# Gorilla-Lab-SCUT/frustum-convnet

Hardware: AMD Instinct MI355X
Metric: frustums/sec (train fwd+bwd) KITTI-car B=32 N=1024 (higher is better)
Workload: dtype f32 (fp32 operands split into two 16-bit parts, 3 MFMAs per product, fp32 accumulate); 1 GPU; cfgs/det_sample.yaml KITTI-car, batch=32/GPU, Npoint=1024, L=(280,140,70,35), train fwd+bwd+Adam; global_batch=32, parallelism=dp1

## Files before the change

frustum_convnet_amd/_native.py:

```python
import ctypes
import os

_HERE = os.path.dirname(os.path.abspath(__file__))
LIB_PATH = os.path.join(_HERE, os.environ.get("FCN_LIB_NAME", "libfcn_hip.so"))

c_fp = ctypes.c_void_p

BN_RUNNING = 0
BN_TRAIN = 1
BN_FROZEN = 2


class PnDesc(ctypes.Structure):
    _fields_ = [("B", ctypes.c_int32), ("N", ctypes.c_int32), ("L", ctypes.c_int32), ("K", ctypes.c_int32),
                ("C1", ctypes.c_int32), ("C2", ctypes.c_int32), ("C3", ctypes.c_int32),
                ("nvec", ctypes.c_int32), ("training", ctypes.c_int32),
                ("eps", ctypes.c_float), ("momentum", ctypes.c_float), ("nlc", ctypes.c_int32),
                ("precision", ctypes.c_int32), ("grouped", ctypes.c_int32)]


CN_MAXLEV = 5
CN_MAXLAYER = 18


# ... 4 lines not shown
                ("precision", ctypes.c_int32), ("nlev", ctypes.c_int32), ("c1", ctypes.c_int32)]


class CnParams(ctypes.Structure):
    _fields_ = [("W", c_fp * CN_MAXLAYER), ("gamma", c_fp * CN_MAXLAYER), ("beta", c_fp * CN_MAXLAYER),
                ("running_mean", c_fp * CN_MAXLAYER), ("running_var", c_fp * CN_MAXLAYER),
                ("num_batches_tracked", c_fp * CN_MAXLAYER), ("bias", c_fp)]


class CnWs(ctypes.Structure):
    _fields_ = [("y", c_fp), ("dz", c_fp), ("wp", c_fp), ("bn", c_fp), ("stat", c_fp), ("bstat", c_fp),
                ("coef", c_fp), ("partial", c_fp), ("oh64", c_fp), ("flags", c_fp)]


class PnParams(ctypes.Structure):
    _fields_ = [("W", c_fp * 3), ("gamma", c_fp * 3), ("beta", c_fp * 3),
                ("running_mean", c_fp * 3), ("running_var", c_fp * 3), ("num_batches_tracked", c_fp * 3)]


class PnWs(ctypes.Structure):
    _fields_ = [("woff", c_fp), ("ent", c_fp), ("ewin", c_fp), ("tiles", c_fp), ("y2", c_fp), ("y3", c_fp), ("amax", c_fp),
                ("stat", c_fp), ("bn", c_fp), ("gmax", c_fp), ("dy3", c_fp), ("dz2", c_fp), ("bstat", c_fp),
                ("coef", c_fp), ("partial", c_fp), ("nsplit", ctypes.c_int32), ("gmom", c_fp), ("wenc", c_fp), ("flags", c_fp), ("pkey", c_fp),
                ("partial_both", ctypes.c_int32)]


class PnInferWs(ctypes.Structure):
    _fields_ = [("w1f", c_fp), ("wenc", c_fp), ("shift", c_fp)]


class InpDesc(ctypes.Structure):
    _fields_ = [("B", ctypes.c_int32), ("N", ctypes.c_int32), ("pt_stride", ctypes.c_int32), ("L", ctypes.c_int32 * 4),
                ("stride", ctypes.c_double * 4), ("max_depth", ctypes.c_double),
                ("random_flip", ctypes.c_int32), ("random_shift", ctypes.c_int32)]


class Inp5Desc(ctypes.Structure):
    _fields_ = [("B", ctypes.c_int32), ("N", ctypes.c_int32), ("pt_stride", ctypes.c_int32), ("L", ctypes.c_int32 * 5),
                ("stride", ctypes.c_double * 5), ("max_depth", ctypes.c_double),
                ("random_flip", ctypes.c_int32), ("random_shift", ctypes.c_int32)]


class InpRefineDesc(ctypes.Structure):
    _fields_ = [("B", ctypes.c_int32), ("N", ctypes.c_int32), ("pt_stride", ctypes.c_int32), ("Lpad", ctypes.c_int32 * 4),
                ("stride", ctypes.c_double * 4), ("random_flip", ctypes.c_int32), ("random_shift", ctypes.c_int32)]


# ... 225 lines not shown
```

frustum_convnet_amd/csrc/group_compact.hip:

```cpp
#include "fcn_common.h"
#include "pn_pack.h"

#define GC_T 256
#define GC_WAVES (GC_T / 64)
#ifndef GC_WPB
#define GC_WPB 16
#endif
#define GC_MAX_SCALES 8
#define GC_LDS_MAX_PTS 8192
#define GC_MOM 12

struct GcScale {
    const float *ref;
    float dis_z;
    int L, K, C1, C2, C3;
    int32_t *woff, *ewin, *tiles, *cnt;
    float4 *ent;
    unsigned short *ghits;
    double *stat;
    double *gmom;
    const float *W1, *gamma, *beta;
    float *rmean, *rvar;
    int64_t *nbt;
    float *bn1;
// ... 4 lines not shown
    PackArgs pk[GC_MAX_SCALES];
    const float *pc;
    int B, N, use_lds;
    int batch_stats;
    float eps, momentum;
    int fold;
};

#define GE_T 1024
#define GE_WAVES (GE_T / 64)

__device__ __forceinline__ GcScale gc_pick(const GcArgs &a, int z)
{
    GcScale S = a.s[0];
#pragma unroll
    for (int q = 1; q < GC_MAX_SCALES; ++q)
        if (z == q) S = a.s[q];
    return S;
}


__device__ __forceinline__ void gc_fold_bn1(const GcArgs &a, const GcScale &S, const double *mo, int tid, int nthr)
{
    const double M = (double)a.B * (double)S.L * (double)S.K;
    for (int c = tid; c < S.C1; c += nthr) {
        double mean, var;
        if (a.batch_stats) {
            const double iM = 1.0 / M;
            const double mx = mo[1] * iM, my = mo[2] * iM, mz = mo[3] * iM;
            const double cxx = mo[4] * iM - mx * mx, cxy = mo[5] * iM - mx * my, cxz = mo[6] * iM - mx * mz;
            const double cyy = mo[7] * iM - my * my, cyz = mo[8] * iM - my * mz, czz = mo[9] * iM - mz * mz;
            const double w0 = S.W1[3 * c], w1 = S.W1[3 * c + 1], w2 = S.W1[3 * c + 2];
            mean = w0 * mx + w1 * my + w2 * mz;
            var = w0 * (cxx * w0 + cxy * w1 + cxz * w2) + w1 * (cxy * w0 + cyy * w1 + cyz * w2) +
                  w2 * (cxz * w0 + cyz * w1 + czz * w2);
            if (var < 0.0) var = 0.0;
            if (S.rmean) {
                S.rmean[c] = (float)((1.0 - a.momentum) * S.rmean[c] + a.momentum * mean);
                S.rvar[c] = (float)((1.0 - a.momentum) * S.rvar[c] + a.momentum * var * (M / (M - 1.0)));
                if (c == 0 && S.nbt) S.nbt[0] += 1;
            }
        } else {
            mean = S.rmean[c];
            var = S.rvar[c];
        }
        const double rstd = fcn_rsqrt64(var + (double)a.eps);
        const double sc = (double)S.gamma[c] * rstd;
        S.bn1[c] = (float)sc;
        S.bn1[S.C1 + c] = (float)((double)S.beta[c] - mean * sc);
        S.bn1[2 * S.C1 + c] = (float)mean;
        S.bn1[3 * S.C1 + c] = (float)rstd;
    }
}

__global__ __launch_bounds__(GC_T) void gc_hits_kernel(GcArgs a)
{
    FCN_DYN_LDS(unsigned char, smem);
    const int tid = threadIdx.x, lane = tid & 63, wave = tid >> 6;
    const int b = blockIdx.y;
    const GcScale S = gc_pick(a, (int)blockIdx.z);
    const int L = S.L, K = S.K, N = a.N;
    {
        PackArgs P = a.pk[0];
#pragma unroll
        for (int q = 1; q < GC_MAX_SCALES; ++q)
            if ((int)blockIdx.z == q) P = a.pk[q];
        if (P.wenc) pn_pack_range(P, ((int)blockIdx.y * (int)gridDim.x + (int)blockIdx.x) * GC_T + tid, (int)(gridDim.x * gridDim.y) * GC_T);
    }
    if ((int)blockIdx.x * GC_WPB >= L) return;
    float *zs = (float *)smem;
    const float *pz = a.pc + (int64_t)b * 3 * N + 2 * (int64_t)N;
    if (a.use_lds) {
        for (int i = tid; i < N; i += GC_T) zs[i] = pz[i];
        __syncthreads();
// ... 256 lines not shown
```

frustum_convnet_amd/csrc/pn_pack.h:

```cpp
#pragma once
#include "gemm_tile.h"

__host__ __device__ inline int64_t pn_wenc_off(int img, int C1, int C2, int C3)
{
    const int64_t a = (int64_t)C2 * C1, b = (int64_t)C3 * C2;
    return img == 0 ? 0 : (img == 1 ? a : (img == 2 ? a + b : 2 * a + b));
}
__host__ __device__ inline int64_t pn_wenc_floats(int C1, int C2, int C3) { return 2 * ((int64_t)C2 * C1 + (int64_t)C3 * C2); }

template <int MM>
__device__ __forceinline__ void pn_pack_item(const float *__restrict__ W, int COUT, int CIN, bool grad, int t, u32x4 *__restrict__ img)
{
    const int NC = grad ? CIN : COUT;
    const int n = t % NC, r = t / NC, kb = r & 3, c = r >> 2;
    float x[8];
    if (!grad) {
        const v4f a = ldg4(W + (int64_t)n * CIN + c * KC + 8 * kb), b = ldg4(W + (int64_t)n * CIN + c * KC + 8 * kb + 4);
        x[0] = a.x; x[1] = a.y; x[2] = a.z; x[3] = a.w; x[4] = b.x; x[5] = b.y; x[6] = b.z; x[7] = b.w;
    } else {
#pragma unroll
        for (int j = 0; j < 8; ++j) x[j] = W[(int64_t)(c * KC + 8 * kb + j) * CIN + n];
    }
    u32x4 hi, lo;
    enc8<MM>(x, hi, lo);
    img[((int64_t)c * 8 + kb) * NC + n] = hi;
    img[((int64_t)c * 8 + 4 + kb) * NC + n] = lo;
}

struct PackArgs {
    const float *W2, *W3;
    float *wenc;
    int C1, C2, C3, precision;
};

__device__ __forceinline__ void pn_pack_range(const PackArgs &a, int first, int step)
{
    const int n2 = a.C2 * a.C1 / 8, n3 = a.C3 * a.C2 / 8;
    u32x4 *F2 = (u32x4 *)(a.wenc + pn_wenc_off(0, a.C1, a.C2, a.C3)), *F3 = (u32x4 *)(a.wenc + pn_wenc_off(1, a.C1, a.C2, a.C3));
    u32x4 *G2 = (u32x4 *)(a.wenc + pn_wenc_off(2, a.C1, a.C2, a.C3)), *G3 = (u32x4 *)(a.wenc + pn_wenc_off(3, a.C1, a.C2, a.C3));
    const int mmf = FCN_MM_OF(a.precision, true), mmb = FCN_MM_OF(a.precision, false);
    for (int t = first; t < 2 * (n2 + n3); t += step) {
        const bool grad = t >= n2 + n3;
        const int u = grad ? t - (n2 + n3) : t;
        const bool l3 = u >= n2;
        const int v = l3 ? u - n2 : u;
        const float *W = l3 ? a.W3 : a.W2;
        const int COUT = l3 ? a.C3 : a.C2, CIN = l3 ? a.C2 : a.C1;
        u32x4 *img = grad ? (l3 ? G3 : G2) : (l3 ? F3 : F2);
        const int mm = grad ? mmb : mmf;
        if (mm == MM_F32) pn_pack_item<MM_F32>(W, COUT, CIN, grad, v, img);
        else if (mm == MM_F16X3) pn_pack_item<MM_F16X3>(W, COUT, CIN, grad, v, img);
// ... 6 lines not shown
```

frustum_convnet_amd/csrc/pointnet_fwd.hip:

```cpp
#define FCN_TUNING_PNF
#include "gemm_tile.h"

#define LDT 129
#define MAXC 512
#ifndef FCN_WIDE_TILES
#define FCN_WIDE_TILES 0
#endif
#ifndef FCN_C3_BIG
#define FCN_C3_BIG 1
#endif
#ifndef FCN_FWD_EPI_DIRECT
#define FCN_FWD_EPI_DIRECT 0
#endif

__global__ void bn1_finalize_kernel(const double *__restrict__ mom, const float *__restrict__ W1,
                                    const float *__restrict__ gamma, const float *__restrict__ beta,
                                    float *rmean, float *rvar, int64_t *nbt, int C, int batch_stats,
                                    float eps, float momentum, double M, float *__restrict__ bn)
{
    const int c = blockIdx.x * blockDim.x + threadIdx.x;
    if (c >= C) return;
    double mean, var;
    if (batch_stats) {
        const double mx = mom[1] / M, my = mom[2] / M, mz = mom[3] / M;
// ... 110 lines not shown
    const float4 *ent;
    const int32_t *woff;
    const int32_t *tiles;
    const float *aprev;
    const float *bn_in;
    const float *W1;
    const u32x4 *Wenc;
    int32_t *flags;
    float *y;
    double *stat;
    int save_y;
    int L, cap, CIN, COUT, tps;
    const double *stat_in;
    int rep_stride;
    const float *gamma_in, *beta_in;
    float *rmean_in, *rvar_in;
    int64_t *nbt_in;
    float *bn_pub;
    double M;
    float eps, momentum;
    const int32_t *ewin;
    unsigned long long *pkey;
    const float *gamma_out;
};

__device__ __forceinline__ void fwd_bn_in(const FwdArgs &a, int i, bool pub, float &fs, float &ft, bool have = false, double s1 = 0.0,
                                          double s2 = 0.0)
{
    const int C = a.CIN;
    double mean, var;
    if (a.stat_in) {
        const double invM = 1.0 / a.M;
        if (!have) {
            s1 = fcn_rep_sum(a.stat_in + i, a.rep_stride);
            s2 = fcn_rep_sum(a.stat_in + C + i, a.rep_stride);
        }
        mean = s1 * invM;
        var = s2 * invM - mean * mean;
        if (var < 0.0) var = 0.0;
    } else {
        mean = a.rmean_in[i];
        var = a.rvar_in[i];
    }
    const double rstd = fcn_rsqrt64(var + (double)a.eps);
    const double sc = (double)a.gamma_in[i] * rstd;
    fs = (float)sc;
    ft = (float)((double)a.beta_in[i] - mean * sc);
    if (pub) {
        a.bn_pub[i] = fs; a.bn_pub[C + i] = ft; a.bn_pub[2 * C + i] = (float)mean; a.bn_pub[3 * C + i] = (float)rstd;
        if (a.stat_in && a.rmean_in) {
            a.rmean_in[i] = (float)((1.0 - a.momentum) * a.rmean_in[i] + a.momentum * mean);
            a.rvar_in[i] = (float)((1.0 - a.momentum) * a.rvar_in[i] + a.momentum * var * (a.M / (a.M - 1.0)));
            if (i == 0 && a.nbt_in) a.nbt_in[0] += 1;
        }
    }
}

template <int MM, int MODE, int NT, int WN, int MT = 2, int POOL = 0>
__global__ __launch_bounds__(128 * WN) __attribute__((amdgpu_waves_per_eu(MT == 1 ? 4 : 3, 4))) void fwd_gemm_kernel(FwdArgs a)
{
    constexpr int NTHR = 128 * WN;
    constexpr int TM = 64 * MT;
    constexpr int SUB = 128 / TM;
    constexpr int TN = 32 * NT * WN;
    constexpr int LDRA = KbTile<TM>::LDR, LDRB = KbTile<TN>::LDR;
    constexpr int NA4 = TM * 8 / NTHR;
    constexpr int NB = TN * 8 / NTHR;
    constexpr int KBT = 4 * TM / NTHR;
    constexpr int OPU4 = KbTile<TM>::U4 + KbTile<TN>::U4, EPU4 = (NTHR / 64) * EP_FLOATS / 4;
    constexpr int LDSU4 = OPU4 > EPU4 ? OPU4 : EPU4;
    __shared__ u32x4 lds4[LDSU4];
    __shared__ __attribute__((aligned(16))) float tS[MAXC];
    __shared__ __attribute__((aligned(16))) float sS[MODE == 0 ? 3 * MAXC : MAXC];
    __shared__ float wS[TM];
    __shared__ int winS[POOL ? TM : 1], insS[POOL ? 64 : 1];
    u32x4 *Ab = lds4, *Bb = lds4 + KbTile<TM>::U4;

    const int tid = threadIdx.x, lane = tid & 63, wave = tid >> 6;
    const int l31 = lane & 31, lh = lane >> 5;
    const int wm = wave / WN, wn = wave % WN;
    const int ny = a.COUT / TN;
    if constexpr (MODE == 1) {
        if (blockIdx.x == 0 && a.gamma_in) {
            for (int i = tid; i < a.CIN; i += NTHR) {
                float fs, ft;
                fwd_bn_in(a, i, true, fs, ft);
            }
        }
    }
    double q1[FCN_STAT_REP], q2[FCN_STAT_REP];
    const bool early = FCN_EARLY_STATS && MODE == 1 && a.gamma_in && a.stat_in && tid < a.CIN;
    if constexpr (MODE == 1) {
        if (early) {
#pragma unroll
            for (int r = 0; r < FCN_STAT_REP; ++r) {
                q1[r] = a.stat_in[(int64_t)r * a.rep_stride + tid];
                q2[r] = a.stat_in[(int64_t)r * a.rep_stride + a.CIN + tid];
            }
        }
        FCN_LOAD_FENCE();
    }
    const int xt = fcn_xcd_tile(blockIdx.x, SUB * a.tiles[0] * ny);
    if (xt < 0) return;
    const int bxi = xt / ny, byi = xt % ny;
    const int lt = bxi / SUB, sub = bxi % SUB;
    const int code = a.tiles[4 + lt];
    const int b = code / a.tps, t = code % a.tps;
    const int nent = a.woff[(int64_t)b * (a.L + 1) + a.L];
    const int row0 = t * 128 + sub * TM;
    const int nvalid = min(TM, nent - row0);
    if (nvalid <= 0) return;
    const int64_t grow0 = (int64_t)b * a.cap + row0;
    const int n0 = byi * TN;
    const int CIN = a.CIN, COUT = a.COUT;

    PNF_DECL;
    u32x4 rw[NB];
    v4f ra[MODE == 1 ? NA4 : 1];
    const u32x4 *wsrc = a.Wenc + n0 + (tid % TN) + (int64_t)(tid / TN) * COUT;
    auto load_chunk = [&](int c) __attribute__((always_inline)) {
        if constexpr (MODE == 1) {
            if (!((FCN_X & 1) && c > 0))
#pragma unroll
            for (int i = 0; i < NA4; ++i) {
                const int f = tid + NTHR * i;
                const int r = f >> 3, kq = f & 7;
                ra[i] = lds4e<MM>(a.aprev, ((int)grow0 + min(r, nvalid - 1)) * CIN + c * KC + 4 * kq);
            }
        }
        if (!((FCN_X & 2) && c > 0))
#pragma unroll
        for (int i = 0; i < NB; ++i) rw[i] = ldgu4(wsrc + ((int64_t)c * 8 + i * (NTHR / TN)) * COUT);
    };
    load_chunk(0);

    for (int i = tid; i < CIN; i += NTHR) {
        float s, t;
        if (MODE == 1 && a.gamma_in) {
            if (early && i == tid) {
                double s1 = q1[0], s2 = q2[0];
#pragma unroll
                for (int r = 1; r < FCN_STAT_REP; ++r) { s1 += q1[r]; s2 += q2[r]; }
                fwd_bn_in(a, i, false, s, t, true, s1, s2);
            } else {
                fwd_bn_in(a, i, false, s, t);
            }
        } else {
            s = a.bn_in[i];
            t = a.bn_in[CIN + i];
        }
        tS[i] = t;
        if constexpr (MODE == 0) {
            sS[3 * i] = s * a.W1[3 * i];
            sS[3 * i + 1] = s * a.W1[3 * i + 1];
            sS[3 * i + 2] = s * a.W1[3 * i + 2];
        } else {
            sS[i] = s;
        }
    }
    if (tid < TM) wS[tid] = (tid < nvalid) ? a.ent[grow0 + tid].w : 0.f;
    int pw = -1, plo = 0, phi = 0;
// ... 31 lines not shown
                const v4f s4 = *(const v4f *)(sS + c * KC + 4 * kq), t4 = *(const v4f *)(tS + c * KC + 4 * kq);
                const float z0 = fcn_relu_keep(fmaf(s4.x, ra[i].x, t4.x), kp), z1 = fcn_relu_keep(fmaf(s4.y, ra[i].y, t4.y), kp);
                const float z2 = fcn_relu_keep(fmaf(s4.z, ra[i].z, t4.z), kp), z3 = fcn_relu_keep(fmaf(s4.w, ra[i].w, t4.w), kp);
                kb_store4<MM_ENC_A, LDRA>(Aq, r, kq, z0, z1, z2, z3);
            }
        } else {
            const int part = tid / TM;
#pragma unroll
            for (int q = 0; q < KBT; ++q) {
                const int kb = part * KBT + q;
                float z[8];
#pragma unroll
                for (int j = 0; j < 8; ++j) {
                    const int kk = c * KC + 8 * kb + j;
                    const float zz = l1_pre(&sS[3 * kk], tS[kk], ux, uy, uz);
                    z[j] = fcn_relu_keep(zz, r0keep);
                }
                u32x4 hi, lo;
                enc8<MM_ENC_A>(z, hi, lo);
                Aq[kb * LDRA + r0] = hi;
                Aq[(4 + kb) * LDRA + r0] = lo;
            }
        }
#pragma unroll
        for (int i = 0; i < NB; ++i) {
            const int f = tid + NTHR * i;
            Bq[(f / TN) * LDRB + (f % TN)] = rw[i];
        }
    };

    PNF_ADD(0);
    for (int c = 0; c < nchunk; ++c) {
        if (!((FCN_X & 4) && c > 0)) stage_chunk(c, Ab, Bb);
        PNF_ADD(2);
        __syncthreads();
        PNF_ADD(3);
        if (c + 1 < nchunk) load_chunk(c + 1);
        PNF_ADD(1);
        if (!(FCN_X & 8)) mma_chunk_kb<MM, MT, NT, LDRA, LDRB>(Ab, Bb, wm * 32 * MT, wn * 32 * NT, acc);
        PNF_ADD(4);
        __syncthreads();
        PNF_ADD(3);
    }

    if (FCN_X & 16) { if (acc[0][0][0] == 123.456f) a.y[0] = 0.f; return; }
    bool bad = false;
    const bool store_y = !POOL || a.save_y;
#if FCN_FWD_EPI_DIRECT
#pragma unroll
    for (int mt = 0; mt < MT; ++mt)
// ... 373 lines not shown
        int ao[2];
#pragma unroll
        for (int e = 0; e < 2; ++e) {
            int row;
            const float y = fcn_pool_key_value(hi[e], lo[e], g[e], row);
            const float u = fmaf(s[e], y, t[e]);
            const bool pos = live && (hi[e] | lo[e]) != 0u && u > 0.f;
            fo[e] = pos ? u : 0.f;
            ao[e] = pos ? row : -1;
            yo[e] = y;
            if (ywin && y3 && g[e] == 0.f && pos) {
                const int64_t yi = ((int64_t)b * cap + row) * C3 + c + e;
                yo[e] = s16 ? __uint_as_float((unsigned)((const unsigned short *)y3)[yi] << 16) : ((const float *)y3)[yi];
            }
        }
        *(v2f *)(feat + o) = v2f{fo[0], fo[1]};
        if (amax) { amax[o] = ao[0]; amax[o + 1] = ao[1]; }
        if (ywin) *(v2f *)(ywin + o) = v2f{yo[0], yo[1]};
    }
}

static inline unsigned pad8(unsigned n) { return (n + 7u) / 8u * 8u; }

template <int MM, int MODE, int POOL>
static int launch_fwd_gemm_mm(const FwdArgs &a, int B, hipStream_t st)
{
    const unsigned nt = (unsigned)(B * a.tps);
    if (FCN_WIDE_TILES && a.COUT % 256 == 0) {
        hipLaunchKernelGGL((fwd_gemm_kernel<MM, MODE, 2, 4, 2, POOL>), dim3(pad8(nt * (a.COUT / 256))), dim3(512), 0, st, a);
    } else if (!FCN_C3_BIG && MODE == 1 && a.COUT >= 512 && a.COUT % 128 == 0) {
        hipLaunchKernelGGL((fwd_gemm_kernel<MM, MODE, 2, 2, 1, POOL>), dim3(pad8(2 * nt * (a.COUT / 128))), dim3(256), 0, st, a);
    } else if (a.COUT % 128 == 0) {
        hipLaunchKernelGGL((fwd_gemm_kernel<MM, MODE, 2, 2, 2, POOL>), dim3(pad8(nt * (a.COUT / 128))), dim3(256), 0, st, a);
    } else {
        hipLaunchKernelGGL((fwd_gemm_kernel<MM, MODE, 1, 2, 2, POOL>), dim3(pad8(nt * (a.COUT / 64))), dim3(256), 0, st, a);
    }
    FCN_CHECK_LAUNCH();
    return 0;
}

template <int MODE>
static int launch_fwd_gemm(const FwdArgs &a, int B, int precision, hipStream_t st)
{
    if (a.CIN % 64 || a.COUT % 64 || a.CIN > MAXC) return FCN_E_BADARG;
    if ((int64_t)B * a.cap * (a.CIN > a.COUT ? a.CIN : a.COUT) >= (int64_t)1 << 31) return FCN_E_LIMIT;
    if (precision < 0 || precision > FCN_PREC_BF16_OPS) return FCN_E_BADARG;
    if constexpr (MODE == 1) {
        if (a.pkey) {
            if (!a.ewin || !a.gamma_out) return FCN_E_BADARG;
            FCN_MM_SWITCH(FCN_MM_OF(precision, true), return (launch_fwd_gemm_mm<MM, MODE, 1>(a, B, st)));
            return FCN_E_BADARG;
        }
    }
    FCN_MM_SWITCH(FCN_MM_OF(precision, true), return (launch_fwd_gemm_mm<MM, MODE, 0>(a, B, st)));
    return FCN_E_BADARG;
}

extern "C" int fcn_pn_forward(const fcn_pn_desc *d, const fcn_pn_params *p, const int32_t *cnt,
                              const float *one_hot, const fcn_pn_ws *ws, float *feat, void *stream)
{
    if (!d || !p || !ws || !cnt || !feat || !ws->wenc || !bn_mode_valid(d)) return FCN_E_BADARG;
    if (d->C1 % 64 || d->C2 % 64 || d->C3 % 64 || d->C1 > MAXC || d->C2 > MAXC) return FCN_E_BADARG;
    if (d->nvec > 0 && !one_hot && !d->nlc) return FCN_E_BADARG;
    if (d->nvec * PW > GT) return FCN_E_LIMIT;
    hipStream_t st = (hipStream_t)stream;
    const int B = d->B, L = d->L, K = d->K, C1 = d->C1, C2 = d->C2, C3 = d->C3;
    const int cap = L * K;
    const double M = (double)B * (double)L * (double)K;
    const int tr = uses_batch_stats(d) ? 1 : 0;
    const int sv = saves_for_backward(d) ? 1 : 0;
    if (sv && ws->amax && !ws->gmax && fcn_pn_key_pool(d, ws, C3)) return FCN_E_BADARG;
    float *bn1 = ws->bn + fcn_bn_off(0, C1, C2);
    float *bn2 = ws->bn + fcn_bn_off(1, C1, C2);
    float *bn3 = ws->bn + fcn_bn_off(2, C1, C2);
    double *st2 = ws->stat + FCN_STAT_L2, *st3 = st2 + 2 * C2;

    if (!d->grouped) {
        FCN_TRY(fcn_pn_pack_weights(d, p, ws, stream));
        hipLaunchKernelGGL(bn1_finalize_kernel, dim3((C1 + 63) / 64), dim3(64), 0, st, ws->stat + FCN_STAT_MOM,
                           p->W[0], p->gamma[0], p->beta[0], p->running_mean[0], p->running_var[0],
                           p->num_batches_tracked[0], C1, tr, d->eps, d->momentum, M, bn1);
        FCN_CHECK_LAUNCH();
    }

    FwdArgs a;
    a.ent = (const float4 *)ws->ent; a.woff = ws->woff; a.tiles = ws->tiles; a.L = L; a.cap = cap; a.tps = (cap + 127) / 128;
    a.aprev = nullptr; a.bn_in = bn1; a.W1 = p->W[0]; a.Wenc = (const u32x4 *)(ws->wenc + pn_wenc_off(0, C1, C2, C3)); a.y = ws->y2;
    a.flags = ws->flags;
    a.stat = tr ? st2 : nullptr; a.save_y = sv; a.CIN = C1; a.COUT = C2;
    a.stat_in = nullptr; a.gamma_in = a.beta_in = nullptr; a.rmean_in = a.rvar_in = nullptr; a.nbt_in = nullptr; a.bn_pub = nullptr;
    a.M = M; a.eps = d->eps; a.momentum = d->momentum; a.rep_stride = 2 * C2 + 2 * C3;
    a.ewin = nullptr; a.pkey = nullptr; a.gamma_out = nullptr;
    FCN_TRY(launch_fwd_gemm<0>(a, B, d->precision, st));

    a.aprev = ws->y2; a.bn_in = bn2; a.W1 = nullptr; a.Wenc = (const u32x4 *)(ws->wenc + pn_wenc_off(1, C1, C2, C3)); a.y = ws->y3;
    a.stat = tr ? st3 : nullptr; a.save_y = sv; a.CIN = C2; a.COUT = C3;
    a.stat_in = tr ? st2 : nullptr; a.gamma_in = p->gamma[1]; a.beta_in = p->beta[1];
    a.rmean_in = p->running_mean[1]; a.rvar_in = p->running_var[1]; a.nbt_in = p->num_batches_tracked[1]; a.bn_pub = bn2;
    const bool key_pool = fcn_pn_key_pool(d, ws, C3);
    if (key_pool) { a.ewin = ws->ewin; a.pkey = (unsigned long long *)ws->pkey; a.gamma_out = p->gamma[2]; }
    FCN_TRY(launch_fwd_gemm<1>(a, B, d->precision, st));

    const bool nlc_pool = d->nlc && (C3 == 128 || C3 == 256 || C3 == 512);
    if (!nlc_pool && !key_pool) {
        hipLaunchKernelGGL(bn_finalize_kernel, dim3((C3 + 63) / 64), dim3(64), 0, st, st3, 2 * C2 + 2 * C3, p->gamma[2], p->beta[2],
                           p->running_mean[2], p->running_var[2], p->num_batches_tracked[2], C3, tr, d->eps,
                           d->momentum, M, bn3);
        FCN_CHECK_LAUNCH();
    }

    const int nz = FCN_STAT_REP * (2 * C3 + 2 * C2 + 4 * C1);
    const bool s16 = d->precision == FCN_PREC_BF16;
    if (key_pool) {
        PoolBn pb;
        pb.stat = tr ? st3 : nullptr; pb.rep_stride = 2 * C2 + 2 * C3; pb.gamma = p->gamma[2]; pb.beta = p->beta[2];
        pb.rmean = p->running_mean[2]; pb.rvar = p->running_var[2]; pb.nbt = p->num_batches_tracked[2]; pb.bn = bn3;
// ... 26 lines not shown
                                    sv ? ws->amax : nullptr, L, cap, C3, d->nvec, d->nlc, sv ? ws->bstat : nullptr, nz);
        else hipLaunchKernelGGL(pool_kernel<0>, pgrid, dim3(GT), 0, st, ws->y3, bn3, ws->woff, cnt, one_hot, feat,
                                sv ? ws->amax : nullptr, L, cap, C3, d->nvec, d->nlc, sv ? ws->bstat : nullptr, nz);
    }
    FCN_CHECK_LAUNCH();
    return 0;
}

extern "C" int fcn_pn_conv_fwd(const fcn_pn_desc *d, const fcn_pn_params *p, const fcn_pn_ws *ws, int layer,
                               int with_stats, void *stream)
{
    if (!d || !p || !ws || (layer != 2 && layer != 3) || !ws->wenc) return FCN_E_BADARG;
    hipStream_t st = (hipStream_t)stream;
    const int B = d->B, L = d->L, K = d->K, C1 = d->C1, C2 = d->C2, C3 = d->C3;
    const int cap = L * K;
    double *st2 = ws->stat + FCN_STAT_L2, *st3 = st2 + 2 * C2;
    FwdArgs a;
    a.ent = (const float4 *)ws->ent; a.woff = ws->woff; a.tiles = ws->tiles; a.L = L; a.cap = cap; a.tps = (cap + 127) / 128;
    a.stat_in = nullptr; a.gamma_in = a.beta_in = nullptr; a.rmean_in = a.rvar_in = nullptr; a.nbt_in = nullptr; a.bn_pub = nullptr;
    a.M = 1.0; a.eps = d->eps; a.momentum = d->momentum;
    a.rep_stride = 2 * C2 + 2 * C3;
    a.flags = ws->flags;
    a.ewin = nullptr; a.pkey = nullptr; a.gamma_out = nullptr; a.save_y = 1;
    if (layer == 2) {
        a.aprev = nullptr; a.bn_in = ws->bn + fcn_bn_off(0, C1, C2); a.W1 = p->W[0]; a.Wenc = (const u32x4 *)(ws->wenc + pn_wenc_off(0, C1, C2, C3)); a.y = ws->y2;
        a.stat = with_stats ? st2 : nullptr; a.CIN = C1; a.COUT = C2;
        return launch_fwd_gemm<0>(a, B, d->precision, st);
    }
    a.aprev = ws->y2; a.bn_in = ws->bn + fcn_bn_off(1, C1, C2); a.W1 = nullptr; a.Wenc = (const u32x4 *)(ws->wenc + pn_wenc_off(1, C1, C2, C3)); a.y = ws->y3;
    a.stat = with_stats ? st3 : nullptr; a.CIN = C2; a.COUT = C3;
    return launch_fwd_gemm<1>(a, B, d->precision, st);
}

#include "pn_infer.h"
```

frustum_convnet_amd/det_base.py:

```python
import math

import numpy as np
import os

import torch
import torch.nn as nn
import torch.nn.functional as F

from .config import cfg
from .dataset_info import DATASET_INFO
from .common import Conv1d, Conv2d, DeConv1d, init_params, softmax_focal_loss_ignore, get_accuracy, masked_mean, bn_momentum
from .query_depth_point import QueryDepthPoint
from .pointnet_fused import WorkspacePool, pointnet_pooled, launch_pooled, attach_pooled
from . import box_ops
from . import _native


def _bn_mode(module):
    if getattr(module, "bn_frozen", False):
        return _native.BN_FROZEN
    return _native.BN_TRAIN if module.training else _native.BN_RUNNING


class PointNetModule(nn.Module):
# ... 216 lines not shown

    def forward(self, point_cloud, sample_pc, feat=None, one_hot_vec=None, nlc=False, join=True):
        if one_hot_vec is not None:
            assert self.num_vec == one_hot_vec.shape[1]
        nets = self.nets
        ns = self.num_scales
        self.done_events = None
        mode = self.bn_mode()
        if not (self.concurrent_scales and point_cloud.is_cuda) or os.environ.get("FCN_SERIAL", "0") == "1":
            self.drop_prefetch()
            for net in nets:
                net._pool.bwd_stream = net._pool.bwd_host_pool = None
            return tuple(net.forward_pooled(point_cloud, ref, one_hot_vec, nlc) for net, ref in zip(nets, sample_pc))
        dev = point_cloud.device
        cur = torch.cuda.current_stream(dev)
        streams = self._streams(dev)
        fork = self._fork_event(dev)
        prepared = None
        if self._prefetched is not None and (self._prefetch_is_foreign() or
                                             self._prefetched["key"] != self._front_key(point_cloud, sample_pc, one_hot_vec, nlc,
                                                                                        mode)):
            self.drop_prefetch()
        if self.fused_front:
            from .pointnet_fused import group_compact, launch_prepared
            if self._prefetched is not None:
                self.join_prefetch()
                prepared = self._prefetched["handles"]
                self._prefetched = None
                group_compact(prepared, point_cloud, phase=2)
            else:
                prepared = [nets[s].prepare_pooled(point_cloud, sample_pc[s], one_hot_vec, nlc) for s in range(ns)]
                group_compact(prepared, point_cloud)
        fork.record(cur)
        sts = [streams[i] for i in range(ns - 1)] + [cur]
        self._step_id += 1
        for k in range(ns):
            host = self.bwd_share.get(k) if (self.share_active and mode != _native.BN_RUNNING) else None
            pool = nets[k]._pool
            pool.fwd_step = self._step_id
            pool.bwd_stream = None if host is None else streams[host]
            pool.bwd_host_pool = None if host is None else nets[host]._pool
        handles = [None] * ns
        for s in (ns - 1,) + tuple(range(ns - 2, 1, -1)) + (0, 1):
            if sts[s] is not cur:
                sts[s].wait_event(fork)
            with torch.cuda.stream(sts[s]):
                if prepared is not None:
                    handles[s] = launch_prepared(prepared[s])
                else:
                    handles[s] = nets[s].launch_pooled(point_cloud, sample_pc[s], one_hot_vec, nlc)
        outs = [None] * ns
        done = self._done_events(dev)
# ... 453 lines not shown
```

frustum_convnet_amd/pointnet_fused.py:

```python
import ctypes
import os

import torch

from . import _native
from ._native import PnDesc, PnParams, PnWs, PnInferWs
from .query_depth_point import query_depth_point
from . import precision as _precision


def _mid_launch(B, L, K, C3):
    mode = os.environ.get("FCN_PN_MID", "auto")
    if str(L) in os.environ.get("FCN_PN_MID_L", "").split(","):
        return True
    return mode == "1" or (mode == "auto" and C3 <= 128 and B * L * K <= 300000)


class Workspace:

    def __init__(self, B, N, L, K, C1, C2, C3, device, need_grad, flags=None):
        cap = L * K
        f32, i32, f64 = torch.float32, torch.int32, torch.float64
        dev = device
        self.key = (B, N, L, K, C1, C2, C3, bool(need_grad))
# ... 91 lines not shown
        ws.pool_key = k
        return ws

    def release(self, ws):
        self.free.setdefault(ws.pool_key, []).append(ws)


def _params_struct(Ws, gammas, betas, rmeans, rvars, nbts):
    arr = lambda ts: (ctypes.c_void_p * 3)(*[None if t is None else t.data_ptr() for t in ts])
    return PnParams(arr(Ws), arr(gammas), arr(betas), arr(rmeans), arr(rvars), arr(nbts))


def _acquire(pool, cfgt, pc, ref, one_hot, bufs, plist, need_grad):
    dist, K, training, eps, momentum = cfgt[:5]
    nlc = bool(cfgt[6]) if len(cfgt) > 6 else False
    fuse = bool(cfgt[7]) if len(cfgt) > 7 else False
    W1, g1, b1, W2, g2, b2, W3, g3, b3 = plist
    B, _, N = pc.shape
    Lw = ref.shape[2]
    C1, C2, C3 = W1.shape[0], W2.shape[0], W3.shape[0]
    nvec = 0 if (one_hot is None or nlc) else one_hot.shape[1]
    dev = pc.device
    ws = pool.acquire(B, N, Lw, K, C1, C2, C3, device=dev, need_grad=need_grad)
    desc = PnDesc(B, N, Lw, K, C1, C2, C3, nvec, int(training), eps, momentum, 1 if nlc else 0,
                  _precision.code(), 0)
    rmeans, rvars, nbts = bufs
    Wc = [W1.detach().reshape(C1, 3).contiguous(), W2.detach().reshape(C2, C1).contiguous(),
          W3.detach().reshape(C3, C2).contiguous()]
    gs = [g1.detach().contiguous(), g2.detach().contiguous(), g3.detach().contiguous()]
    bs = [b1.detach().contiguous(), b2.detach().contiguous(), b3.detach().contiguous()]
    params = _params_struct(Wc, gs, bs, rmeans, rvars, nbts)
    oh = None if (one_hot is None or nlc) else one_hot.detach().contiguous().float()
    return {"ws": ws, "desc": desc, "params": params, "Wc": Wc, "gs": gs, "bs": bs, "oh": oh, "nlc": nlc, "nvec": nvec,
            "ref": ref, "dist": float(dist), "dims": (B, Lw, C3), "dev": dev,
            "fused_eval": fuse and fused_eval_supported(int(training), desc.precision, C2),
            "bufs": bufs}


INFER_MAX_C2 = 256


def fused_eval_supported(mode, precision_code, C2):
    if not (int(mode) == _native.BN_RUNNING and precision_code != _precision.CODES["f32"] and C2 <= INFER_MAX_C2):
        return False
    if not hasattr(_native.lib(), "fcn_pn_infer"):
        raise RuntimeError("fuse_eval is on, but the loaded native library has no fcn_pn_infer (built from older kernel "
# ... 35 lines not shown
    B, Lw, C3 = h["dims"]
    dev = h["dev"]
    feat = torch.empty((B, Lw, C3) if h["nlc"] else (B, C3 + h["nvec"], Lw), dtype=torch.float32, device=dev)
    with torch.cuda.device(dev):
        _native.check(L.fcn_pn_forward(ctypes.byref(h["desc"]), ctypes.byref(h["params"]), cnt.data_ptr(),
                                       None if h["oh"] is None else h["oh"].data_ptr(), ctypes.byref(h["ws"].c),
                                       feat.data_ptr(), _native.current_stream(dev)), "fcn_pn_forward")
    return feat, idx, cnt, h["ws"], h["desc"], (h["Wc"], h["gs"], h["bs"], cnt, idx, h["oh"])


def _forward_impl(pool, cfgt, pc, ref, one_hot, bufs, plist, need_grad):
    L = _native.lib()
    h = _acquire(pool, cfgt, pc, ref, one_hot, bufs, plist, need_grad)
    idx, cnt = query_depth_point(h["dist"], h["desc"].K, pc, ref)
    with torch.cuda.device(h["dev"]):
        _native.check(L.fcn_pn_compact(ctypes.byref(h["desc"]), pc.data_ptr(), ref.data_ptr(), idx.data_ptr(),
                                       cnt.data_ptr(), ctypes.byref(h["ws"].c), _native.current_stream(h["dev"])), "fcn_pn_compact")
    if h["fused_eval"]:
        infer_fold([h])
        return _run_infer(h, cnt, idx)
    return _run_forward(h, cnt, idx)


def group_compact(handles, pc, phase=3):
    L = _native.lib()
    n = len(handles)
    dev = pc.device
    phase_all = phase == 3
    fused = all(h.get("fused_eval") for h in handles)
    if not fused:
        for h in handles:
            h["fused_eval"] = False
    elif phase == 2:
        infer_fold(handles)
        return
    elif phase == 3:
        phase = 1
    arr = lambda vals: (ctypes.c_void_p * n)(*vals)
    descs = arr([ctypes.addressof(h["desc"]) for h in handles])
    params = arr([ctypes.addressof(h["params"]) for h in handles])
    refs = arr([h["ref"].data_ptr() for h in handles])
    wss = arr([ctypes.addressof(h["ws"].c) for h in handles])
    cnts = arr([h["ws"].cnt.data_ptr() for h in handles])
    dz = (ctypes.c_float * n)(*[h["dist"] for h in handles])
    with torch.cuda.device(dev):
        _native.check(L.fcn_pn_group_compact2(n, descs, params, pc.data_ptr(), refs, dz, wss, cnts, int(phase),
                                              _native.current_stream(dev)), "fcn_pn_group_compact2")
    if fused:
        if phase_all:
            infer_fold(handles)
        return
    if phase != 1:
        for h in handles:
            h["desc"].grouped = 1


def _empty_idx(dev):
    return torch.empty((0,), dtype=torch.int64, device=dev)


# ... 233 lines not shown
```

include/fcn_hip.h:

```cpp
#ifndef FCN_HIP_H
#define FCN_HIP_H

#include <stdint.h>

#ifdef __cplusplus
extern "C" {
#endif

#define FCN_E_BADARG 10001
#define FCN_E_LIMIT  10002

#define FCN_PREC_SPLIT 0
#define FCN_PREC_F32   1
#define FCN_PREC_BF16  2
#define FCN_PREC_BF16_OPS 3

int fcn_arch(void);

int fcn_query_depth_point_f32(const float *pts_z, int64_t pt_stride, int64_t pt_bstride,
                              const float *ctr_z, int64_t ct_stride, int64_t ct_bstride,
                              int b, int n, int m, float dis_z, int nsample,
                              int64_t *idx, int32_t *cnt, void *stream);

int fcn_query_depth_point_multi_f32(int nscale, const float *pts_z, int64_t pt_stride, int64_t pt_bstride,
// ... 25 lines not shown

typedef struct fcn_pn_ws {
    int32_t *woff;
    float   *ent;
    int32_t *ewin;
    int32_t *tiles;
    float   *y2;
    float   *y3;
    int32_t *amax;
    double  *stat;
    float   *bn;
    float   *gmax;
    float   *dy3;
    float   *dz2;
    double  *bstat;
    float   *coef;
    float   *partial;
    int32_t  nsplit;
    double  *gmom;
    float   *wenc;
    int32_t *flags;
    uint64_t *pkey;
    int32_t  partial_both;
} fcn_pn_ws;

#define FCN_FLAG_NONFINITE 1

int fcn_pn_wgrad_rows(void);
int fcn_stat_replicas(void);

int fcn_pn_compact(const fcn_pn_desc *d, const float *pc , const float *ref ,
                   const int64_t *idx, const int32_t *cnt, const fcn_pn_ws *ws, void *stream);

int fcn_pn_group_compact(int nscale, const fcn_pn_desc *const *d, const fcn_pn_params *const *p, const float *pc,
                         const float *const *ref, const float *dis_z, const fcn_pn_ws *const *ws, int32_t *const *cnt,
                         void *stream);

int fcn_pn_group_compact2(int nscale, const fcn_pn_desc *const *d, const fcn_pn_params *const *p, const float *pc,
                          const float *const *ref, const float *dis_z, const fcn_pn_ws *const *ws, int32_t *const *cnt,
                          int phase, void *stream);

int fcn_pn_pack_weights(const fcn_pn_desc *d, const fcn_pn_params *p, const fcn_pn_ws *ws, void *stream);
int fcn_pn_pack_weights_all(int nscale, const fcn_pn_desc *const *d, const fcn_pn_params *const *p,
                            const fcn_pn_ws *const *ws, void *stream);

int fcn_pn_forward(const fcn_pn_desc *d, const fcn_pn_params *p, const int32_t *cnt,
// ... 256 lines not shown
```

Before: 29490 frustums/s.

## Fold BN1 and weight packing into conv2 GEMM instead of phase-2 group pass

When prefetching is used, the phase-2 group_compact launch is skipped and its work moves into the conv2 forward GEMM. Block 0 of that GEMM folds the conv1 batch-norm statistics into scale and shift and publishes them, and every block recomputes the fold it needs locally. Extra 'rider' blocks appended to the grid pack the W2/W3 split-precision weight images, and conv2 itself reads raw fp32 W2 and encodes it on the fly. This saves a kernel launch and a pass over the weights, at the cost of redundant per-block BN fold math and in-loop encoding. A possible risk is that the rider-packed W3 image has to be ready before conv3 runs.

```diff
diff --git a/frustum_convnet_amd/_native.py b/frustum_convnet_amd/_native.py
--- a/frustum_convnet_amd/_native.py
+++ b/frustum_convnet_amd/_native.py
@@ -50,7 +50,7 @@
     _fields_ = [("woff", c_fp), ("ent", c_fp), ("ewin", c_fp), ("tiles", c_fp), ("y2", c_fp), ("y3", c_fp), ("amax", c_fp),
                 ("stat", c_fp), ("bn", c_fp), ("gmax", c_fp), ("dy3", c_fp), ("dz2", c_fp), ("bstat", c_fp),
                 ("coef", c_fp), ("partial", c_fp), ("nsplit", ctypes.c_int32), ("gmom", c_fp), ("wenc", c_fp), ("flags", c_fp), ("pkey", c_fp),
-                ("partial_both", ctypes.c_int32)]
+                ("partial_both", ctypes.c_int32), ("fold_in_conv2", ctypes.c_int32)]
 
 
 class PnInferWs(ctypes.Structure):
diff --git a/frustum_convnet_amd/csrc/group_compact.hip b/frustum_convnet_amd/csrc/group_compact.hip
--- a/frustum_convnet_amd/csrc/group_compact.hip
+++ b/frustum_convnet_amd/csrc/group_compact.hip
@@ -50,34 +50,13 @@
 
 __device__ __forceinline__ void gc_fold_bn1(const GcArgs &a, const GcScale &S, const double *mo, int tid, int nthr)
 {
-    const double M = (double)a.B * (double)S.L * (double)S.K;
+    Bn1Fold f;
+    f.W1 = S.W1; f.gamma = S.gamma; f.beta = S.beta; f.rmean = S.rmean; f.rvar = S.rvar; f.nbt = S.nbt; f.bn1 = S.bn1;
+    f.C1 = S.C1; f.batch_stats = a.batch_stats; f.eps = a.eps; f.momentum = a.momentum;
+    f.M = (double)a.B * (double)S.L * (double)S.K;
     for (int c = tid; c < S.C1; c += nthr) {
-        double mean, var;
-        if (a.batch_stats) {
-            const double iM = 1.0 / M;
-            const double mx = mo[1] * iM, my = mo[2] * iM, mz = mo[3] * iM;
-            const double cxx = mo[4] * iM - mx * mx, cxy = mo[5] * iM - mx * my, cxz = mo[6] * iM - mx * mz;
-            const double cyy = mo[7] * iM - my * my, cyz = mo[8] * iM - my * mz, czz = mo[9] * iM - mz * mz;
-            const double w0 = S.W1[3 * c], w1 = S.W1[3 * c + 1], w2 = S.W1[3 * c + 2];
-            mean = w0 * mx + w1 * my + w2 * mz;
-            var = w0 * (cxx * w0 + cxy * w1 + cxz * w2) + w1 * (cxy * w0 + cyy * w1 + cyz * w2) +
-                  w2 * (cxz * w0 + cyz * w1 + czz * w2);
-            if (var < 0.0) var = 0.0;
-            if (S.rmean) {
-                S.rmean[c] = (float)((1.0 - a.momentum) * S.rmean[c] + a.momentum * mean);
-                S.rvar[c] = (float)((1.0 - a.momentum) * S.rvar[c] + a.momentum * var * (M / (M - 1.0)));
-                if (c == 0 && S.nbt) S.nbt[0] += 1;
-            }
-        } else {
-            mean = S.rmean[c];
-            var = S.rvar[c];
-        }
-        const double rstd = fcn_rsqrt64(var + (double)a.eps);
-        const double sc = (double)S.gamma[c] * rstd;
-        S.bn1[c] = (float)sc;
-        S.bn1[S.C1 + c] = (float)((double)S.beta[c] - mean * sc);
-        S.bn1[2 * S.C1 + c] = (float)mean;
-        S.bn1[3 * S.C1 + c] = (float)rstd;
+        float fs, ft;
+        pn_bn1_fold(f, mo, c, true, fs, ft);
     }
 }
 
diff --git a/frustum_convnet_amd/csrc/pn_pack.h b/frustum_convnet_amd/csrc/pn_pack.h
--- a/frustum_convnet_amd/csrc/pn_pack.h
+++ b/frustum_convnet_amd/csrc/pn_pack.h
@@ -27,6 +27,51 @@
     img[((int64_t)c * 8 + 4 + kb) * NC + n] = lo;
 }
 
+struct Bn1Fold {
+    const float *W1, *gamma, *beta;
+    float *rmean, *rvar;
+    int64_t *nbt;
+    float *bn1;
+    int C1, batch_stats;
+    float eps, momentum;
+    double M;
+};
+
+__device__ __forceinline__ void pn_bn1_fold(const Bn1Fold &f, const double *mo, int c, bool pub, float &fs, float &ft)
+{
+    const double M = f.M;
+    double mean, var;
+    if (f.batch_stats) {
+        const double iM = 1.0 / M;
+        const double mx = mo[1] * iM, my = mo[2] * iM, mz = mo[3] * iM;
+        const double cxx = mo[4] * iM - mx * mx, cxy = mo[5] * iM - mx * my, cxz = mo[6] * iM - mx * mz;
+        const double cyy = mo[7] * iM - my * my, cyz = mo[8] * iM - my * mz, czz = mo[9] * iM - mz * mz;
+        const double w0 = f.W1[3 * c], w1 = f.W1[3 * c + 1], w2 = f.W1[3 * c + 2];
+        mean = w0 * mx + w1 * my + w2 * mz;
+        var = w0 * (cxx * w0 + cxy * w1 + cxz * w2) + w1 * (cxy * w0 + cyy * w1 + cyz * w2) +
+              w2 * (cxz * w0 + cyz * w1 + czz * w2);
+        if (var < 0.0) var = 0.0;
+        if (pub && f.rmean) {
+            f.rmean[c] = (float)((1.0 - f.momentum) * f.rmean[c] + f.momentum * mean);
+            f.rvar[c] = (float)((1.0 - f.momentum) * f.rvar[c] + f.momentum * var * (M / (M - 1.0)));
+            if (c == 0 && f.nbt) f.nbt[0] += 1;
+        }
+    } else {
+        mean = f.rmean[c];
+        var = f.rvar[c];
+    }
+    const double rstd = fcn_rsqrt64(var + (double)f.eps);
+    const double sc = (double)f.gamma[c] * rstd;
+    fs = (float)sc;
+    ft = (float)((double)f.beta[c] - mean * sc);
+    if (pub) {
+        f.bn1[c] = fs;
+        f.bn1[f.C1 + c] = ft;
+        f.bn1[2 * f.C1 + c] = (float)mean;
+        f.bn1[3 * f.C1 + c] = (float)rstd;
+    }
+}
+
 struct PackArgs {
     const float *W2, *W3;
     float *wenc;
diff --git a/frustum_convnet_amd/csrc/pointnet_fwd.hip b/frustum_convnet_amd/csrc/pointnet_fwd.hip
--- a/frustum_convnet_amd/csrc/pointnet_fwd.hip
+++ b/frustum_convnet_amd/csrc/pointnet_fwd.hip
@@ -156,6 +156,9 @@
     const int32_t *ewin;
     unsigned long long *pkey;
     const float *gamma_out;
+    const float *W;
+    PackArgs pk;
+    int rider0, nrider;
 };
 
 __device__ __forceinline__ void fwd_bn_in(const FwdArgs &a, int i, bool pub, float &fs, float &ft, bool have = false, double s1 = 0.0,
@@ -190,9 +193,10 @@
     }
 }
 
-template <int MM, int MODE, int NT, int WN, int MT = 2, int POOL = 0>
+template <int MM, int MODE, int NT, int WN, int MT = 2, int POOL = 0, int FOLD = 0>
 __global__ __launch_bounds__(128 * WN) __attribute__((amdgpu_waves_per_eu(MT == 1 ? 4 : 3, 4))) void fwd_gemm_kernel(FwdArgs a)
 {
+    static_assert(!FOLD || MODE == 0, "the fold form is conv2's");
     constexpr int NTHR = 128 * WN;
     constexpr int TM = 64 * MT;
     constexpr int SUB = 128 / TM;
@@ -214,6 +218,25 @@
     const int l31 = lane & 31, lh = lane >> 5;
     const int wm = wave / WN, wn = wave % WN;
     const int ny = a.COUT / TN;
+    Bn1Fold f1;
+    double mo[10];
+    if constexpr (FOLD) {
+        if ((int)blockIdx.x >= a.rider0) {
+            pn_pack_range(a.pk, ((int)blockIdx.x - a.rider0) * NTHR + tid, a.nrider * NTHR);
+            return;
+        }
+        f1.W1 = a.W1; f1.gamma = a.gamma_in; f1.beta = a.beta_in; f1.rmean = a.rmean_in; f1.rvar = a.rvar_in; f1.nbt = a.nbt_in;
+        f1.bn1 = a.bn_pub; f1.C1 = a.CIN; f1.batch_stats = a.stat_in ? 1 : 0; f1.eps = a.eps; f1.momentum = a.momentum; f1.M = a.M;
+#pragma unroll
+        for (int i = 0; i < 10; ++i) mo[i] = a.stat_in ? a.stat_in[i] : 0.0;
+        if (blockIdx.x == 0) {
+            for (int i = tid; i < a.CIN; i += NTHR) {
+                float fs, ft;
+                pn_bn1_fold(f1, mo, i, true, fs, ft);
+            }
+        }
+        FCN_LOAD_FENCE();
+    }
     if constexpr (MODE == 1) {
         if (blockIdx.x == 0 && a.gamma_in) {
             for (int i = tid; i < a.CIN; i += NTHR) {
@@ -252,6 +275,8 @@
     u32x4 rw[NB];
     v4f ra[MODE == 1 ? NA4 : 1];
     const u32x4 *wsrc = a.Wenc + n0 + (tid % TN) + (int64_t)(tid / TN) * COUT;
+    static_assert(!FOLD || (NB % 2 == 0 && (NB / 2) * (NTHR / TN) == 4), "a thread's image rows pair up as (hi, lo) of whole items");
+    const float *wraw = FOLD ? a.W + (int64_t)(n0 + tid % TN) * CIN + 8 * (tid / TN) : nullptr;
     auto load_chunk = [&](int c) __attribute__((always_inline)) {
         if constexpr (MODE == 1) {
             if (!((FCN_X & 1) && c > 0))
@@ -262,15 +287,26 @@
                 ra[i] = lds4e<MM>(a.aprev, ((int)grow0 + min(r, nvalid - 1)) * CIN + c * KC + 4 * kq);
             }
         }
+        if constexpr (FOLD) {
+#pragma unroll
+            for (int i = 0; i < NB / 2; ++i) {
+                const u32x4 *src = (const u32x4 *)(wraw + c * KC + 8 * i * (NTHR / TN));
+                rw[2 * i] = ldgu4(src);
+                rw[2 * i + 1] = ldgu4(src + 1);
+            }
+        } else {
         if (!((FCN_X & 2) && c > 0))
 #pragma unroll
         for (int i = 0; i < NB; ++i) rw[i] = ldgu4(wsrc + ((int64_t)c * 8 + i * (NTHR / TN)) * COUT);
+        }
     };
     load_chunk(0);
 
     for (int i = tid; i < CIN; i += NTHR) {
         float s, t;
-        if (MODE == 1 && a.gamma_in) {
+        if constexpr (FOLD) {
+            pn_bn1_fold(f1, mo, i, false, s, t);
+        } else if (MODE == 1 && a.gamma_in) {
             if (early && i == tid) {
                 double s1 = q1[0], s2 = q2[0];
 #pragma unroll
@@ -348,10 +384,23 @@
                 Aq[(4 + kb) * LDRA + r0] = lo;
             }
         }
+        if constexpr (FOLD) {
+#pragma unroll
+            for (int i = 0; i < NB / 2; ++i) {
+                const int kb = tid / TN + i * (NTHR / TN);
+                const v4f x0 = __builtin_bit_cast(v4f, rw[2 * i]), x1 = __builtin_bit_cast(v4f, rw[2 * i + 1]);
+                const float x[8] = {x0.x, x0.y, x0.z, x0.w, x1.x, x1.y, x1.z, x1.w};
+                u32x4 hi, lo;
+                enc8<MM>(x, hi, lo);
+                Bq[kb * LDRB + (tid % TN)] = hi;
+                Bq[(4 + kb) * LDRB + (tid % TN)] = lo;
+            }
+        } else {
 #pragma unroll
         for (int i = 0; i < NB; ++i) {
             const int f = tid + NTHR * i;
             Bq[(f / TN) * LDRB + (f % TN)] = rw[i];
+        }
         }
     };
 
@@ -771,6 +820,25 @@
 
 static inline unsigned pad8(unsigned n) { return (n + 7u) / 8u * 8u; }
 
+template <int MM>
+static int launch_fwd_gemm_fold(FwdArgs a, int B, hipStream_t st)
+{
+    const unsigned nt = (unsigned)(B * a.tps);
+    const int items = 2 * (a.pk.C2 * a.pk.C1 + a.pk.C3 * a.pk.C2) / 8;
+    if (FCN_WIDE_TILES && a.COUT % 256 == 0) {
+        a.rider0 = (int)pad8(nt * (a.COUT / 256)); a.nrider = (items + 511) / 512;
+        hipLaunchKernelGGL((fwd_gemm_kernel<MM, 0, 2, 4, 2, 0, 1>), dim3(a.rider0 + a.nrider), dim3(512), 0, st, a);
+    } else if (a.COUT % 128 == 0) {
+        a.rider0 = (int)pad8(nt * (a.COUT / 128)); a.nrider = (items + 255) / 256;
+        hipLaunchKernelGGL((fwd_gemm_kernel<MM, 0, 2, 2, 2, 0, 1>), dim3(a.rider0 + a.nrider), dim3(256), 0, st, a);
+    } else {
+        a.rider0 = (int)pad8(nt * (a.COUT / 64)); a.nrider = (items + 255) / 256;
+        hipLaunchKernelGGL((fwd_gemm_kernel<MM, 0, 1, 2, 2, 0, 1>), dim3(a.rider0 + a.nrider), dim3(256), 0, st, a);
+    }
+    FCN_CHECK_LAUNCH();
+    return 0;
+}
+
 template <int MM, int MODE, int POOL>
 static int launch_fwd_gemm_mm(const FwdArgs &a, int B, hipStream_t st)
 {
@@ -789,11 +857,17 @@
 }
 
 template <int MODE>
-static int launch_fwd_gemm(const FwdArgs &a, int B, int precision, hipStream_t st)
+static int launch_fwd_gemm(const FwdArgs &a, int B, int precision, hipStream_t st, bool fold = false)
 {
     if (a.CIN % 64 || a.COUT % 64 || a.CIN > MAXC) return FCN_E_BADARG;
     if ((int64_t)B * a.cap * (a.CIN > a.COUT ? a.CIN : a.COUT) >= (int64_t)1 << 31) return FCN_E_LIMIT;
     if (precision < 0 || precision > FCN_PREC_BF16_OPS) return FCN_E_BADARG;
+    if constexpr (MODE == 0) {
+        if (fold) {
+            FCN_MM_SWITCH(FCN_MM_OF(precision, true), return (launch_fwd_gemm_fold<MM>(a, B, st)));
+            return FCN_E_BADARG;
+        }
+    }
     if constexpr (MODE == 1) {
         if (a.pkey) {
             if (!a.ewin || !a.gamma_out) return FCN_E_BADARG;
@@ -819,6 +893,13 @@
     const int tr = uses_batch_stats(d) ? 1 : 0;
     const int sv = saves_for_backward(d) ? 1 : 0;
     if (sv && ws->amax && !ws->gmax && fcn_pn_key_pool(d, ws, C3)) return FCN_E_BADARG;
+    if (ws->fold_in_conv2 < 0 || ws->fold_in_conv2 > 1) return FCN_E_BADARG;
+    const bool fold = ws->fold_in_conv2 == 1;
+    if (fold) {
+        if (!d->grouped || !ws->stat || !ws->bn || ((uintptr_t)ws->wenc & 15)) return FCN_E_BADARG;
+        if (!p->W[0] || !p->W[1] || !p->W[2] || !p->gamma[0] || !p->beta[0]) return FCN_E_BADARG;
+        if (!tr && (!p->running_mean[0] || !p->running_var[0])) return FCN_E_BADARG;
+    }
     float *bn1 = ws->bn + fcn_bn_off(0, C1, C2);
     float *bn2 = ws->bn + fcn_bn_off(1, C1, C2);
     float *bn3 = ws->bn + fcn_bn_off(2, C1, C2);
@@ -840,7 +921,15 @@
     a.stat_in = nullptr; a.gamma_in = a.beta_in = nullptr; a.rmean_in = a.rvar_in = nullptr; a.nbt_in = nullptr; a.bn_pub = nullptr;
     a.M = M; a.eps = d->eps; a.momentum = d->momentum; a.rep_stride = 2 * C2 + 2 * C3;
     a.ewin = nullptr; a.pkey = nullptr; a.gamma_out = nullptr;
-    FCN_TRY(launch_fwd_gemm<0>(a, B, d->precision, st));
+    a.W = nullptr; a.pk.W2 = a.pk.W3 = nullptr; a.pk.wenc = nullptr; a.pk.C1 = C1; a.pk.C2 = C2; a.pk.C3 = C3; a.pk.precision = d->precision;
+    a.rider0 = a.nrider = 0;
+    if (fold) {
+        a.stat_in = tr ? ws->stat + FCN_STAT_MOM : nullptr; a.gamma_in = p->gamma[0]; a.beta_in = p->beta[0];
+        a.rmean_in = p->running_mean[0]; a.rvar_in = p->running_var[0]; a.nbt_in = p->num_batches_tracked[0]; a.bn_pub = bn1;
+        a.W = p->W[1]; a.pk.W2 = p->W[1]; a.pk.W3 = p->W[2]; a.pk.wenc = ws->wenc;
+    }
+    FCN_TRY(launch_fwd_gemm<0>(a, B, d->precision, st, fold));
+    a.W = nullptr; a.pk.wenc = nullptr;
 
     a.aprev = ws->y2; a.bn_in = bn2; a.W1 = nullptr; a.Wenc = (const u32x4 *)(ws->wenc + pn_wenc_off(1, C1, C2, C3)); a.y = ws->y3;
     a.stat = tr ? st3 : nullptr; a.save_y = sv; a.CIN = C2; a.COUT = C3;
@@ -913,6 +1002,7 @@
     a.rep_stride = 2 * C2 + 2 * C3;
     a.flags = ws->flags;
     a.ewin = nullptr; a.pkey = nullptr; a.gamma_out = nullptr; a.save_y = 1;
+    a.W = nullptr; a.pk = PackArgs{}; a.rider0 = a.nrider = 0;
     if (layer == 2) {
         a.aprev = nullptr; a.bn_in = ws->bn + fcn_bn_off(0, C1, C2); a.W1 = p->W[0]; a.Wenc = (const u32x4 *)(ws->wenc + pn_wenc_off(0, C1, C2, C3)); a.y = ws->y2;
         a.stat = with_stats ? st2 : nullptr; a.CIN = C1; a.COUT = C2;
diff --git a/frustum_convnet_amd/det_base.py b/frustum_convnet_amd/det_base.py
--- a/frustum_convnet_amd/det_base.py
+++ b/frustum_convnet_amd/det_base.py
@@ -262,12 +262,12 @@
                                                                                         mode)):
             self.drop_prefetch()
         if self.fused_front:
-            from .pointnet_fused import group_compact, launch_prepared
+            from .pointnet_fused import group_compact, launch_prepared, fold_in_conv2
             if self._prefetched is not None:
                 self.join_prefetch()
                 prepared = self._prefetched["handles"]
                 self._prefetched = None
-                group_compact(prepared, point_cloud, phase=2)
+                group_compact(prepared, point_cloud, phase=2, fold=fold_in_conv2())
             else:
                 prepared = [nets[s].prepare_pooled(point_cloud, sample_pc[s], one_hot_vec, nlc) for s in range(ns)]
                 group_compact(prepared, point_cloud)
diff --git a/frustum_convnet_amd/pointnet_fused.py b/frustum_convnet_amd/pointnet_fused.py
--- a/frustum_convnet_amd/pointnet_fused.py
+++ b/frustum_convnet_amd/pointnet_fused.py
@@ -137,6 +137,7 @@
     nvec = 0 if (one_hot is None or nlc) else one_hot.shape[1]
     dev = pc.device
     ws = pool.acquire(B, N, Lw, K, C1, C2, C3, device=dev, need_grad=need_grad)
+    ws.c.fold_in_conv2 = 0
     desc = PnDesc(B, N, Lw, K, C1, C2, C3, nvec, int(training), eps, momentum, 1 if nlc else 0,
                   _precision.code(), 0)
     rmeans, rvars, nbts = bufs
@@ -218,7 +219,11 @@
     return _run_forward(h, cnt, idx)
 
 
-def group_compact(handles, pc, phase=3):
+def fold_in_conv2():
+    return os.environ.get("FCN_FOLD_IN_CONV2", "1") != "0"
+
+
+def group_compact(handles, pc, phase=3, fold=False):
     L = _native.lib()
     n = len(handles)
     dev = pc.device
@@ -232,6 +237,11 @@
         return
     elif phase == 3:
         phase = 1
+    if phase == 2 and fold:
+        for h in handles:
+            h["ws"].c.fold_in_conv2 = 1
+            h["desc"].grouped = 1
+        return
     arr = lambda vals: (ctypes.c_void_p * n)(*vals)
     descs = arr([ctypes.addressof(h["desc"]) for h in handles])
     params = arr([ctypes.addressof(h["params"]) for h in handles])
diff --git a/include/fcn_hip.h b/include/fcn_hip.h
--- a/include/fcn_hip.h
+++ b/include/fcn_hip.h
@@ -71,6 +71,7 @@
     int32_t *flags;
     uint64_t *pkey;
     int32_t  partial_both;
+    int32_t  fold_in_conv2;
 } fcn_pn_ws;
 
 #define FCN_FLAG_NONFINITE 1
```

Result: slower. 29170 frustums/s (-1.1%).
